# davawen/Simple-Raytracer

Measured on AMD Instinct MI355X. Metric: Mray/s at 1920x1080x1024spp, higher is better.
Workload: dtype f32; 1 GPU; BASELINE configs[1]: 7-shape sphere scene 1920x1080 1024spp; width=1920, height=1080, spp=1024, bounces=10, triangles=12, partition=single GPU, gather=none, mode=parity (fp-contract off, IEEE div/sqrt; canvas bit-identical to the CPU oracle)

## Files before the change

### include/srt_abi.h

```cpp
#ifndef SRT_ABI_H
#define SRT_ABI_H

#include "srt_types.h"

#ifdef __cplusplus
extern "C" {
#endif

typedef struct srt_tracer srt_tracer;

enum {
	SRT_OK = 0,
	SRT_ERR_INVALID = 1,
	SRT_ERR_HIP = 2,
	SRT_ERR_STATE = 3
};

typedef struct srt_counters {
	uint64_t paths;
	uint64_t rays;
	uint64_t sky;
	uint64_t tri_tests;
	uint64_t tri_pass_u;
	uint64_t nan_pixels;
// ... 254 lines not shown
int srt_group_read_bloom(srt_group *g, int level, float *rgba_out, size_t cap_pixels, int *w, int *h);
int srt_last_resolve_bloomed(const srt_tracer *t, int *bloomed);
int srt_group_last_resolve_bloomed(const srt_group *g, int *bloomed);

#define SRT_NOISE_EIGHTHS {0x1.000000p+0f, 0x1.172b84p+0f, 0x1.306fe0p+0f, 0x1.4bfdaep+0f, 0x1.6a09e6p+0f, 0x1.8ace54p+0f, 0x1.ae89fap+0f, 0x1.d5818ep+0f}
int srt_noise_defaults(srt_noise_params *out);
int srt_noise_check_host(const srt_noise_params *p);
int srt_noise_evaluate_host(const uint32_t hist[256], const uint32_t counts[3], uint32_t T, uint32_t P, const srt_noise_params *params, srt_noise_result *result);
int srt_set_noise_meter(srt_tracer *t, const srt_noise_params *p);
int srt_group_set_noise_meter(srt_group *g, const srt_noise_params *p);
int srt_meter_noise(srt_tracer *t);
int srt_group_meter_noise(srt_group *g);
int srt_poll_noise(srt_tracer *t, srt_noise_result *result, uint32_t hist[256], int *ready);
int srt_read_noise(srt_tracer *t, srt_noise_result *result, uint32_t hist[256]);
int srt_group_poll_noise(srt_group *g, srt_noise_result *result, uint32_t hist[256], int *ready);
int srt_group_read_noise(srt_group *g, srt_noise_result *result, uint32_t hist[256]);
int srt_resolve_noise_view(srt_tracer *t);
int srt_group_resolve_noise_view(srt_group *g);
int srt_group_read_noise_view(srt_group *g, uint8_t *argb_out);
int srt_render_until(srt_tracer *t, const srt_render_data *options, uint32_t time_stride, uint32_t max_dispatches, uint8_t *argb_out,
                     srt_noise_result *result, uint32_t *dispatches_done);
int srt_last_meter_ran(const srt_tracer *t, int *ran);
int srt_selftest_noise_meter(srt_tracer *t, const float *canvas_host, const float *moments_host, uint32_t num_pixels, uint32_t T, uint32_t P,
                             const srt_noise_params *params, uint32_t hist_out[256], uint32_t counts_out[3], uint8_t *view_out);


int srt_cast_rays(srt_tracer *t, const srt_ray *rays, size_t n, uint32_t flags, srt_ray_hit *hits);
int srt_cast_rays_device(srt_tracer *t, const void *rays_dev, size_t n, uint32_t flags, void *hits_dev);
int srt_pick(srt_tracer *t, const srt_render_data *options, const float *xy, size_t n, srt_ray_hit *hits);
int srt_group_cast_rays(srt_group *g, const srt_ray *rays, size_t n, uint32_t flags, srt_ray_hit *hits);
int srt_group_pick(srt_group *g, const srt_render_data *options, const float *xy, size_t n, srt_ray_hit *hits);
int srt_last_ray_query_ms(srt_tracer *t, float *ms);
int srt_ray_query_sizes(size_t out[2]);


int srt_occluded_rays(srt_tracer *t, const srt_ray *rays, size_t n, uint32_t flags, uint64_t *occluded, uint64_t *invalid );
int srt_occluded_rays_device(srt_tracer *t, const void *rays_dev, size_t n, uint32_t flags, void *occluded_dev, void *invalid_dev );
int srt_occluded_segments(srt_tracer *t, const srt_segment *segs, size_t n, uint64_t *occluded, uint64_t *invalid );
int srt_segment_rays(srt_tracer *t, const srt_segment *segs, size_t n, srt_ray *rays_out);
int srt_group_occluded_rays(srt_group *g, const srt_ray *rays, size_t n, uint32_t flags, uint64_t *occluded, uint64_t *invalid);
int srt_group_occluded_segments(srt_group *g, const srt_segment *segs, size_t n, uint64_t *occluded, uint64_t *invalid);
int srt_group_segment_rays(srt_group *g, const srt_segment *segs, size_t n, srt_ray *rays_out);
int srt_occlusion_sizes(size_t out[2]);

int srt_selftest_math(srt_tracer *t, uint32_t stride, uint64_t out[16]);

int srt_selftest_rare_lanes(srt_tracer *t, int what, const uint32_t *in, uint32_t waves, uint32_t *out_new, uint32_t *out_ref, uint64_t *mismatches);

int srt_selftest_plane_forms(srt_tracer *t, int what, const float planes[32], const float cam_org[3], const uint32_t *in, uint32_t waves,
                             uint32_t *out_new, uint32_t *out_ref, uint32_t *fast, uint64_t *mismatches);

int srt_selftest_diffuse_bounce(srt_tracer *t, const uint32_t *in, uint32_t waves, uint32_t *out_new, uint32_t *out_ref, uint32_t *fast, uint64_t *mismatches);

int srt_selection_defaults(srt_selection_params *out);
int srt_selection_check_host(const srt_selection_params *p);
int srt_selection_sizes(size_t out[1]);
int srt_selection_alpha_table_host(const srt_selection_params *p, uint8_t *table, size_t cap, int *radius);
int srt_set_selection(srt_tracer *t, const srt_selection_params *p, const uint32_t *shapes, size_t n);
int srt_group_set_selection(srt_group *g, const srt_selection_params *p, const uint32_t *shapes, size_t n);
int srt_render_ids(srt_tracer *t, const srt_render_data *options);
int srt_read_id_pass(srt_tracer *t, uint32_t *shape, uint32_t *triangle, int32_t *material, size_t cap_pixels, int *w, int *h);
int srt_group_read_id_pass(srt_group *g, uint32_t *shape, uint32_t *triangle, int32_t *material, size_t cap_pixels, int *w, int *h);
int srt_read_selection_alpha(srt_tracer *t, uint8_t *alpha, size_t cap_pixels);
int srt_last_resolve_selected(const srt_tracer *t, int *applied, int *id_pass_ran);
int srt_group_last_resolve_selected(const srt_group *g, int *applied, int *id_pass_ran);

const char *srt_version(void);

#ifdef __cplusplus
}
#endif

#endif
```

### simple-raytracer_amd/csrc/frame.hip

```cpp
#include <hip/hip_runtime.h>

#include "device_math.h"
#include "tonemap.h"

namespace {
__device__ __forceinline__ float add_lum2(float s2, float r, float g, float b) {
	const float l = lum(r, g, b);
	return s2 + l * l;
}
}
template <bool MOMENTS>
__global__ __launch_bounds__(256) void srt_reduce_kernel(const ReduceParams p) {
	const uint32_t q = blockIdx.x * blockDim.x + threadIdx.x;
	if (q == 0u && p.queue_reset) *p.queue_reset = 0ull;
	if (q >= p.num_pixels) return;
	f3 c = mk(0.f, 0.f, 0.f);
	float s2 = 0.f;
	float4 *run = reinterpret_cast<float4 *>(p.running) + q;
	if (!p.first_batch) {
		float4 v = *run;
		c = mk(v.x, v.y, v.z);
		if (MOMENTS) s2 = v.w;
	}
	const uint32_t n = p.batch_samples;
	const float *__restrict__ r = p.radiance + (size_t)q * n * 3u;
	uint32_t k = 0;
	if ((n & 3u) == 0u) {
		const float4 *__restrict__ r4 = reinterpret_cast<const float4 *>(r);
#ifndef SRT_REDUCE_DEPTH
#define SRT_REDUCE_DEPTH 4
#endif
		for (; k + 4 * SRT_REDUCE_DEPTH <= n; k += 4 * SRT_REDUCE_DEPTH) {
			float4 v[3 * SRT_REDUCE_DEPTH];
#pragma unroll
			for (int i = 0; i < 3 * SRT_REDUCE_DEPTH; i++) v[i] = r4[i];
			r4 += 3 * SRT_REDUCE_DEPTH;
#pragma unroll
			for (int i = 0; i < 3 * SRT_REDUCE_DEPTH; i += 3) {
				const float4 a = v[i], b = v[i + 1], d = v[i + 2];
				c = c + mk(a.x, a.y, a.z);
				if (MOMENTS) s2 = add_lum2(s2, a.x, a.y, a.z);
				c = c + mk(a.w, b.x, b.y);
				if (MOMENTS) s2 = add_lum2(s2, a.w, b.x, b.y);
				c = c + mk(b.z, b.w, d.x);
				if (MOMENTS) s2 = add_lum2(s2, b.z, b.w, d.x);
				c = c + mk(d.y, d.z, d.w);
				if (MOMENTS) s2 = add_lum2(s2, d.y, d.z, d.w);
			}
		}
		for (; k < n; k += 4) {
			const float4 a = r4[0], b = r4[1], d = r4[2];
			r4 += 3;
			c = c + mk(a.x, a.y, a.z);
			if (MOMENTS) s2 = add_lum2(s2, a.x, a.y, a.z);
			c = c + mk(a.w, b.x, b.y);
			if (MOMENTS) s2 = add_lum2(s2, a.w, b.x, b.y);
			c = c + mk(b.z, b.w, d.x);
			if (MOMENTS) s2 = add_lum2(s2, b.z, b.w, d.x);
			c = c + mk(d.y, d.z, d.w);
			if (MOMENTS) s2 = add_lum2(s2, d.y, d.z, d.w);
		}
	} else {
		for (; k < n; k++) {
			c = c + mk(r[3 * k], r[3 * k + 1], r[3 * k + 2]);
			if (MOMENTS) s2 = add_lum2(s2, r[3 * k], r[3 * k + 1], r[3 * k + 2]);
		}
	}
	if (p.last_batch) {
		c = c / (float)p.num_samples;
		float4 *out = reinterpret_cast<float4 *>(p.canvas) + q;
		float4 o = *out;
		o.x += c.x;
		o.y += c.y;
		o.z += c.z;
		*out = o;
		if (c.x != c.x || c.y != c.y || c.z != c.z) atomicAdd(&p.counters[SRT_CTR_NAN], 1ull);
		if (!MOMENTS && p.argb) {
			const float n = (float)p.num_steps;
			const float r = sqrt_ieee(aces1(o.x / n)), g = sqrt_ieee(aces1(o.y / n)), b = sqrt_ieee(aces1(o.z / n));
			reinterpret_cast<uint32_t *>(p.argb)[q] = 255u | (to_uchar(r * 255.0f) << 8) | (to_uchar(g * 255.0f) << 16) | (to_uchar(b * 255.0f) << 24);
		}
		if (MOMENTS) p.moments[q] += s2 / (float)p.num_samples;
	} else {
		*run = make_float4(c.x, c.y, c.z, MOMENTS ? s2 : 0.f);
	}
}

__global__ __launch_bounds__(256) void srt_prepass_kernel(const PrepassParams p) {
	const int si = blockIdx.y;
	if (si >= p.num_shapes) return;
	const srt_shape *sh = p.shapes + si;
	if (sh->type != SRT_SHAPE_MODEL) return;
	const srt_model *m = &sh->shape.model;
	const uint32_t n = m->num_triangles;
	const uint32_t base = p.wtri_offset[si];
	for (uint32_t s = blockIdx.x * blockDim.x + threadIdx.x; s < n; s += gridDim.x * blockDim.x) {
		const uint32_t j = p.order ? p.order[base + s] : s;
		const srt_triangle *t = p.triangles + (m->triangle_index + j);
		f3 p0 = mat_by_vec(m->transform, ld3(t->vertices[0].pos), 1.0f);
		f3 p1 = mat_by_vec(m->transform, ld3(t->vertices[1].pos), 1.0f);
		f3 p2 = mat_by_vec(m->transform, ld3(t->vertices[2].pos), 1.0f);
		f3 e1 = p1 - p0, e2 = p2 - p0;
		float *w = p.order ? p.wtris + (size_t)(p.dest[base + s] >> 2) * 32u + (p.dest[base + s] & 3u) * SRT_BVH_TRI_FLOATS
		                   : p.wtris + (size_t)(base + s) * SRT_WTRI_FLOATS;
		w[0] = p0.x, w[1] = p0.y, w[2] = p0.z;
		w[3] = e1.x, w[4] = e1.y, w[5] = e1.z;
		w[6] = e2.x, w[7] = e2.y, w[8] = e2.z;
		if (p.order) p.wtris[(size_t)(p.dest[base + s] >> 2) * 32u + SRT_BVH_LEAF_J + (p.dest[base + s] & 3u)] = dm_u2f(j);
	}
}


__global__ __launch_bounds__(256) void srt_resolve_kernel(const ResolveParams p) {
	const float4 *__restrict__ canvas = reinterpret_cast<const float4 *>(p.canvas);
	uint32_t *__restrict__ out = reinterpret_cast<uint32_t *>(p.argb);
	const float n = (float)p.num_steps;
	for (uint32_t i = blockIdx.x * blockDim.x + threadIdx.x; i < p.num_pixels; i += gridDim.x * blockDim.x) {
		float4 c = canvas[i];
		float r = sqrt_ieee(aces1(c.x / n));
		float g = sqrt_ieee(aces1(c.y / n));
		float b = sqrt_ieee(aces1(c.z / n));
		out[i] = 255u | (to_uchar(r * 255.0f) << 8) | (to_uchar(g * 255.0f) << 16) | (to_uchar(b * 255.0f) << 24);
	}
}

void srt_launch_reduce(const ReduceParams &p, void *stream) {
	if (p.num_pixels == 0) return;
	hipLaunchKernelGGL(srt_reduce_kernel<false>, dim3((p.num_pixels + 255) / 256), dim3(256), 0, (hipStream_t)stream, p);
}

void srt_launch_prepass(const PrepassParams &p, uint64_t max_tris_per_model, void *stream) {
	if (p.num_shapes <= 0 || max_tris_per_model == 0) return;
	unsigned gx = (unsigned)((max_tris_per_model + 255) / 256);
	if (gx > 4096) gx = 4096;
	dim3 grid(gx, (unsigned)p.num_shapes), block(256);
	hipLaunchKernelGGL(srt_prepass_kernel, grid, block, 0, (hipStream_t)stream, p);
}

void srt_launch_resolve(const ResolveParams &p, void *stream) {
	if (p.num_pixels == 0) return;
	unsigned gx = (p.num_pixels + 255) / 256;
	if (gx > 4096) gx = 4096;
	hipLaunchKernelGGL(srt_resolve_kernel, dim3(gx), dim3(256), 0, (hipStream_t)stream, p);
}

void srt_launch_reduce_moments(const ReduceParams &p, void *stream) {
	if (p.num_pixels == 0) return;
	hipLaunchKernelGGL(srt_reduce_kernel<true>, dim3((p.num_pixels + 255) / 256), dim3(256), 0, (hipStream_t)stream, p);
}
```

### simple-raytracer_amd/csrc/srt_abi.hip

```cpp
#include <hip/hip_runtime.h>

#include <cstdlib>
#include <cstring>
#include <new>
#include <string>
#include <vector>

#include "../../include/srt_abi.h"
#include "detmath.h"
#include "device_types.h"

#include "scene_prep.h"
#include "srt_internal.h"
#include "trace_plan.h"

namespace {

thread_local std::string g_create_error;

int num_blocks(int height, int rpb) { return (height + rpb - 1) / rpb; }

int clear_canvas_impl(srt_tracer *t) {
	const int rc = srt_temporal_commit(t);
	if (rc) return rc;
// ... 1004 lines not shown
	if (!planes || !cam_org || !in || !out_new || !out_ref || !fast || !mismatches || what < 0 || what > 1 || waves == 0 || waves > 65536u)
		return fail(t, SRT_ERR_INVALID, "srt_selftest_plane_forms: bad arguments");
	SRT_HIP(t, hipSetDevice(t->device));
	const size_t lanes = (size_t)waves * 64u, in_bytes = lanes * 8u * sizeof(uint32_t), out_bytes = lanes * 2u * sizeof(uint32_t), fast_bytes = (size_t)waves * sizeof(uint32_t);
	char *d = nullptr;
	SRT_HIP(t, hipMalloc(reinterpret_cast<void **>(&d), in_bytes + 2 * out_bytes + sizeof(unsigned long long) + fast_bytes));
	uint32_t *d_in = reinterpret_cast<uint32_t *>(d), *d_new = reinterpret_cast<uint32_t *>(d + in_bytes), *d_ref = reinterpret_cast<uint32_t *>(d + in_bytes + out_bytes);
	unsigned long long *d_bad = reinterpret_cast<unsigned long long *>(d + in_bytes + 2 * out_bytes), h_bad = 0;
	uint32_t *d_fast = reinterpret_cast<uint32_t *>(d + in_bytes + 2 * out_bytes + sizeof(unsigned long long));
	hipError_t e = hipMemcpyAsync(d_in, in, in_bytes, hipMemcpyHostToDevice, t->stream);
	if (e == hipSuccess) e = hipMemsetAsync(d_new, 0, 2 * out_bytes + sizeof(unsigned long long) + fast_bytes, t->stream);
	if (e == hipSuccess) {
		srt_launch_selftest_plane_forms(what, planes, cam_org, d_in, waves, d_new, d_ref, d_fast, d_bad, t->stream);
		e = hipGetLastError();
	}
	if (e == hipSuccess) e = hipMemcpyAsync(out_new, d_new, out_bytes, hipMemcpyDeviceToHost, t->stream);
	if (e == hipSuccess) e = hipMemcpyAsync(out_ref, d_ref, out_bytes, hipMemcpyDeviceToHost, t->stream);
	if (e == hipSuccess) e = hipMemcpyAsync(fast, d_fast, fast_bytes, hipMemcpyDeviceToHost, t->stream);
	if (e == hipSuccess) e = hipMemcpyAsync(&h_bad, d_bad, sizeof h_bad, hipMemcpyDeviceToHost, t->stream);
	if (e == hipSuccess) e = hipStreamSynchronize(t->stream);
	(void)hipFree(d);
	if (e != hipSuccess) return fail(t, SRT_ERR_HIP, std::string("srt_selftest_plane_forms: ") + hipGetErrorString(e));
	*mismatches = h_bad;
	return SRT_OK;
}

int srt_selftest_diffuse_bounce(srt_tracer *t, const uint32_t *in, uint32_t waves, uint32_t *out_new, uint32_t *out_ref, uint32_t *fast, uint64_t *mismatches) {
	if (!t) return SRT_ERR_INVALID;
	if (!in || !out_new || !out_ref || !fast || !mismatches || waves == 0 || waves > 65536u) return fail(t, SRT_ERR_INVALID, "srt_selftest_diffuse_bounce: bad arguments");
	SRT_HIP(t, hipSetDevice(t->device));
	const size_t lanes = (size_t)waves * 64u, in_bytes = lanes * 20u * sizeof(uint32_t), out_bytes = lanes * 8u * sizeof(uint32_t), fast_bytes = (size_t)waves * sizeof(uint32_t);
	char *d = nullptr;
	SRT_HIP(t, hipMalloc(reinterpret_cast<void **>(&d), in_bytes + 2 * out_bytes + sizeof(unsigned long long) + fast_bytes));
	uint32_t *d_in = reinterpret_cast<uint32_t *>(d), *d_new = reinterpret_cast<uint32_t *>(d + in_bytes), *d_ref = reinterpret_cast<uint32_t *>(d + in_bytes + out_bytes);
	unsigned long long *d_bad = reinterpret_cast<unsigned long long *>(d + in_bytes + 2 * out_bytes), h_bad = 0;
	uint32_t *d_fast = reinterpret_cast<uint32_t *>(d + in_bytes + 2 * out_bytes + sizeof(unsigned long long));
	hipError_t e = hipMemcpyAsync(d_in, in, in_bytes, hipMemcpyHostToDevice, t->stream);
	if (e == hipSuccess) e = hipMemsetAsync(d_new, 0, 2 * out_bytes + sizeof(unsigned long long) + fast_bytes, t->stream);
	if (e == hipSuccess) {
		srt_launch_selftest_diffuse_bounce(d_in, waves, d_new, d_ref, d_fast, d_bad, t->stream);
		e = hipGetLastError();
	}
	if (e == hipSuccess) e = hipMemcpyAsync(out_new, d_new, out_bytes, hipMemcpyDeviceToHost, t->stream);
	if (e == hipSuccess) e = hipMemcpyAsync(out_ref, d_ref, out_bytes, hipMemcpyDeviceToHost, t->stream);
	if (e == hipSuccess) e = hipMemcpyAsync(fast, d_fast, fast_bytes, hipMemcpyDeviceToHost, t->stream);
	if (e == hipSuccess) e = hipMemcpyAsync(&h_bad, d_bad, sizeof h_bad, hipMemcpyDeviceToHost, t->stream);
	if (e == hipSuccess) e = hipStreamSynchronize(t->stream);
	(void)hipFree(d);
	if (e != hipSuccess) return fail(t, SRT_ERR_HIP, std::string("srt_selftest_diffuse_bounce: ") + hipGetErrorString(e));
	*mismatches = h_bad;
	return SRT_OK;
}

int srt_debug_counters(srt_tracer *t, uint64_t out[18]) {
	if (!t || !out) return SRT_ERR_INVALID;
	SRT_HIP(t, hipSetDevice(t->device));
	std::vector<unsigned long long> w;
	if (const int rc = read_wave_counters(t, w, nullptr)) return rc;
	for (int k = 0; k < 18; k++) out[k] = 0;
	for (size_t i = 0; i < (size_t)2 * SRT_WAVE_CTR_SLOTS; i++) {
		for (int k = 0; k < 8; k++) out[k] += w[i * SRT_WAVE_CTR_STRIDE + k];
		for (int k = 8; k < 16; k++) out[k + 2] += w[i * SRT_WAVE_CTR_STRIDE + k];
	}
	out[8] = (uint64_t)t->last_waves_per_cu;
	out[9] = (uint64_t)t->last_grid;
	return SRT_OK;
}

int srt_debug_region_counters(srt_tracer *t, uint64_t *out, int capacity, int *written) {
	if (!t || !out || !written || capacity < 0) return SRT_ERR_INVALID;
	*written = 0;
#ifdef SRT_REGION_COUNT
	SRT_HIP(t, hipSetDevice(t->device));
	std::vector<unsigned long long> w;
	if (const int rc = read_wave_counters(t, w, nullptr)) return rc;
	const int n = capacity < 2 * SRT_REGION_MAX ? capacity : 2 * SRT_REGION_MAX;
	for (int k = 0; k < n; k++) out[k] = 0;
	for (size_t i = 0; i < (size_t)2 * SRT_WAVE_CTR_SLOTS; i++)
		for (int k = 0; k < n; k++) out[k] += w[i * SRT_WAVE_CTR_STRIDE + 16 + k];
	*written = n;
#endif
	return SRT_OK;
}

int srt_set_count_triangles(srt_tracer *t, int enable) {
	if (!t) return SRT_ERR_INVALID;
	t->count_tris = enable != 0;
	return SRT_OK;
}

}

TraceParams srt_trace_params_for_query(const srt_tracer *t, const srt_render_data *options) { return trace_params_of(t, options, false); }
```

### simple-raytracer_amd/tracer.py

```python
import ctypes as C
from pathlib import Path

import numpy as np

from . import build as B
from . import records as R

PKG = Path(__file__).resolve().parent
import os

LIB_PATH = Path(os.environ["SRT_LIB"]) if os.environ.get("SRT_LIB") else PKG / "lib" / "libsrt_hip.so"

ABI_SYMBOLS = [
    "srt_create", "srt_destroy", "srt_last_error", "srt_set_skybox", "srt_update_scene", "srt_clear_canvas",
    "srt_render", "srt_render_async", "srt_trace", "srt_set_radiance_budget", "srt_resolve", "srt_resolve_external", "srt_synchronize", "srt_read_canvas", "srt_read_argb",
    "srt_get_counters", "srt_set_count_triangles", "srt_reset_counters", "srt_last_kernel_ms", "srt_set_kernel_timers", "srt_last_trace_kernel_ms", "srt_last_trace_launches",
    "srt_device_buffers", "srt_bind_canvas", "srt_bind_stream", "srt_set_partition",
    "srt_partition_owned_rows", "srt_partition_padded_rows", "srt_partition_global_row",
    "srt_partition_unpermute", "srt_selftest_math", "srt_selftest_rare_lanes", "srt_version", "srt_set_acceleration", "srt_acceleration_info", "srt_bvh_build_host", "srt_bvh_wide_host", "srt_debug_counters", "srt_debug_region_counters",
    "srt_comm_unique_id", "srt_comm_init", "srt_gather", "srt_resolve_gathered", "srt_gathered_buffers", "srt_read_gathered",
    "srt_group_create", "srt_group_destroy", "srt_group_last_error", "srt_group_size", "srt_group_tracer", "srt_group_set_skybox",
    "srt_group_set_acceleration", "srt_group_update_scene", "srt_group_clear_canvas", "srt_group_trace_and_gather", "srt_group_render",
    "srt_group_read_canvas", "srt_group_get_counters", "srt_render_pipelined", "srt_pipeline_flush", "srt_unpermute_device",
    "srt_denoise_defaults", "srt_set_denoise", "srt_resolve_denoised", "srt_read_denoised", "srt_read_denoise_inputs",
    "srt_temporal_defaults", "srt_set_denoise_temporal", "srt_reset_denoise_history", "srt_read_denoise_history",
    "srt_set_denoise_object_motion", "srt_read_denoise_shape_ids", "srt_read_denoise_motion", "srt_motion_table_host",
    "srt_set_denoise_vertex_motion", "srt_read_denoise_triangle_ids", "srt_read_denoise_vertex_tables", "srt_motion_table_deform_host",
    "srt_set_textures", "srt_set_material_textures", "srt_set_triangle_uvs", "srt_last_trace_textured", "srt_plane_frame_host",
    "srt_texture_check_host", "srt_group_set_textures", "srt_group_set_material_textures", "srt_group_set_triangle_uvs",
    "srt_last_trace_class", "srt_bernoulli_threshold_host",
    "srt_last_trace_plane_form", "srt_plane_axis_code_host", "srt_selftest_plane_forms", "srt_selftest_diffuse_bounce",
    "srt_set_triangle_materials", "srt_group_set_triangle_materials", "srt_triangle_materials_check_host",
    "srt_group_set_denoise", "srt_group_set_denoise_temporal", "srt_group_reset_denoise_history", "srt_group_resolve_denoised",
    "srt_group_read_denoised", "srt_group_read_denoise_inputs", "srt_group_read_denoise_history", "srt_partition_planes_floats",
    "srt_unpermute_planes_device",
    "srt_set_denoise_demodulation", "srt_group_set_denoise_demodulation", "srt_last_filter_demodulated",
    "srt_group_last_filter_demodulated",
    "srt_set_denoise_spatial_variance", "srt_group_set_denoise_spatial_variance", "srt_last_filter_spatial_variance",
    "srt_group_last_filter_spatial_variance",
    "srt_set_denoise_history_illumination", "srt_group_set_denoise_history_illumination", "srt_last_setup_history_illumination",
    "srt_group_last_setup_history_illumination",
    "srt_set_denoise_history_clamp", "srt_group_set_denoise_history_clamp", "srt_last_setup_history_clamp",
    "srt_group_last_setup_history_clamp", "srt_read_denoise_history_bounds",
    "srt_set_denoise_history_feedback", "srt_group_set_denoise_history_feedback", "srt_last_filter_history_feedback",
    "srt_group_last_filter_history_feedback",
    "srt_bvh_refit_wide_host", "srt_set_acceleration_refit", "srt_group_set_acceleration_refit", "srt_acceleration_refit_info",
    "srt_last_refit_kernel_ms", "srt_read_bvh_blocks", "srt_bvh_wide_order_host",
    "srt_set_acceleration_deform", "srt_group_set_acceleration_deform", "srt_acceleration_deform_info",
    "srt_bvh_refit_deformed_wide_host", "srt_bvh_wide_cost_host",
    "srt_set_acceleration_build", "srt_group_set_acceleration_build", "srt_acceleration_build_info", "srt_last_build_kernel_ms",
    "srt_bvh_morton_order_host", "srt_bvh_morton_wide_host",
    "srt_set_acceleration_build_order", "srt_group_set_acceleration_build_order", "srt_bvh_median_order_host", "srt_bvh_median_wide_host",
    "srt_exposure_defaults", "srt_exposure_check_host", "srt_set_exposure", "srt_group_set_exposure", "srt_reset_exposure",
    "srt_group_reset_exposure", "srt_read_exposure", "srt_group_read_exposure", "srt_last_resolve_exposed",
    "srt_group_last_resolve_exposed",
    "srt_bloom_defaults", "srt_bloom_check_host", "srt_set_bloom", "srt_group_set_bloom", "srt_read_bloom", "srt_group_read_bloom",
    "srt_last_resolve_bloomed", "srt_group_last_resolve_bloomed",
    "srt_noise_defaults", "srt_noise_check_host", "srt_noise_evaluate_host", "srt_set_noise_meter", "srt_group_set_noise_meter",
    "srt_meter_noise", "srt_group_meter_noise", "srt_poll_noise", "srt_group_poll_noise", "srt_read_noise", "srt_group_read_noise",
    "srt_resolve_noise_view", "srt_group_resolve_noise_view", "srt_group_read_noise_view", "srt_render_until", "srt_last_meter_ran",
    "srt_selftest_noise_meter",
    "srt_cast_rays", "srt_cast_rays_device", "srt_pick", "srt_group_cast_rays", "srt_group_pick", "srt_last_ray_query_ms",
    "srt_ray_query_sizes",
    "srt_occluded_rays", "srt_occluded_rays_device", "srt_occluded_segments", "srt_segment_rays", "srt_group_occluded_rays",
    "srt_group_occluded_segments", "srt_group_segment_rays", "srt_occlusion_sizes",
    "srt_selection_defaults", "srt_selection_check_host", "srt_selection_sizes", "srt_selection_alpha_table_host", "srt_set_selection",
    "srt_group_set_selection", "srt_render_ids", "srt_read_id_pass", "srt_group_read_id_pass", "srt_read_selection_alpha",
    "srt_last_resolve_selected", "srt_group_last_resolve_selected",
]

ACCEL_NONE, ACCEL_BVH = 0, 1
REFIT_HOST, REFIT_DEVICE = 0, 1
DEFORM_REBUILD, DEFORM_REFIT = 0, 1
BUILD_HOST, BUILD_DEVICE = 0, 1
BUILD_ORDER_MORTON, BUILD_ORDER_MEDIAN = 0, 1
BUILD_LOCAL = 1024
MOTION_STATIC, MOTION_MOVED, MOTION_NO_HISTORY, MOTION_DEFORMED = 0, 1, 2, 3
MOTION_WORDS = 22
NO_SHAPE = 0xFFFFFFFF
FILTER_LINEAR, FILTER_NEAREST = 0, 1
MAX_TEXTURES = 64


class TextureDesc(C.Structure):
# ... 598 lines not shown
        lib.srt_read_denoise_triangle_ids.argtypes = [vp, vp, vp]
        lib.srt_read_denoise_vertex_tables.argtypes = [vp, vp, vp, sz, C.POINTER(sz)]
        lib.srt_motion_table_deform_host.argtypes = [vp, sz, vp, sz, vp, sz, vp] * 2 + [vp, C.POINTER(C.c_int)]
    if hasattr(lib, "srt_set_denoise_demodulation"):
        lib.srt_set_denoise_demodulation.argtypes = [vp, C.c_int]
        lib.srt_group_set_denoise_demodulation.argtypes = [vp, C.c_int]
        lib.srt_last_filter_demodulated.argtypes = [vp, C.POINTER(C.c_int)]
        lib.srt_group_last_filter_demodulated.argtypes = [vp, C.POINTER(C.c_int)]
    if hasattr(lib, "srt_set_denoise_spatial_variance"):
        lib.srt_set_denoise_spatial_variance.argtypes = [vp, C.c_uint32]
        lib.srt_group_set_denoise_spatial_variance.argtypes = [vp, C.c_uint32]
        lib.srt_last_filter_spatial_variance.argtypes = [vp, C.POINTER(C.c_int)]
        lib.srt_group_last_filter_spatial_variance.argtypes = [vp, C.POINTER(C.c_int)]
    if hasattr(lib, "srt_set_denoise_history_illumination"):
        lib.srt_set_denoise_history_illumination.argtypes = [vp, C.c_int]
        lib.srt_group_set_denoise_history_illumination.argtypes = [vp, C.c_int]
        lib.srt_last_setup_history_illumination.argtypes = [vp]
        lib.srt_group_last_setup_history_illumination.argtypes = [vp]
    if hasattr(lib, "srt_set_denoise_history_clamp"):
        lib.srt_set_denoise_history_clamp.argtypes = [vp, C.c_float]
        lib.srt_group_set_denoise_history_clamp.argtypes = [vp, C.c_float]
        lib.srt_last_setup_history_clamp.argtypes = [vp]
        lib.srt_group_last_setup_history_clamp.argtypes = [vp]
        lib.srt_read_denoise_history_bounds.argtypes = [vp, vp, vp]
    if hasattr(lib, "srt_set_denoise_history_feedback"):
        lib.srt_set_denoise_history_feedback.argtypes = [vp, C.c_int]
        lib.srt_group_set_denoise_history_feedback.argtypes = [vp, C.c_int]
        lib.srt_last_filter_history_feedback.argtypes = [vp]
        lib.srt_group_last_filter_history_feedback.argtypes = [vp]
    if hasattr(lib, "srt_set_textures"):
        lib.srt_set_textures.argtypes = [vp, vp, sz]
        lib.srt_set_material_textures.argtypes = [vp, vp, sz]
        lib.srt_set_triangle_uvs.argtypes = [vp, vp, sz]
        lib.srt_last_trace_textured.argtypes = [vp, C.POINTER(C.c_int)]
        lib.srt_plane_frame_host.argtypes = [vp, vp, vp]
        lib.srt_texture_check_host.argtypes = [vp, sz, vp, sz, C.c_longlong, sz]
        lib.srt_group_set_textures.argtypes = [vp, vp, sz]
        lib.srt_group_set_material_textures.argtypes = [vp, vp, sz]
        lib.srt_group_set_triangle_uvs.argtypes = [vp, vp, sz]
    if hasattr(lib, "srt_set_triangle_materials"):
        lib.srt_set_triangle_materials.argtypes = [vp, vp, sz]
        lib.srt_group_set_triangle_materials.argtypes = [vp, vp, sz]
        lib.srt_triangle_materials_check_host.argtypes = [vp, sz, sz, sz]
    if hasattr(lib, "srt_last_trace_class"):
        lib.srt_last_trace_class.argtypes = [vp, C.POINTER(C.c_int)]
    if hasattr(lib, "srt_last_trace_plane_form"):
        lib.srt_last_trace_plane_form.argtypes = [vp, C.POINTER(C.c_int)]
        lib.srt_plane_axis_code_host.argtypes = [vp, vp, C.POINTER(C.c_int)]
        u32p = C.POINTER(C.c_uint32)
        lib.srt_selftest_plane_forms.argtypes = [vp, i, vp, vp, u32p, C.c_uint32, u32p, u32p, u32p, C.POINTER(C.c_uint64)]
    if hasattr(lib, "srt_selftest_diffuse_bounce"):
        u32p = C.POINTER(C.c_uint32)
        lib.srt_selftest_diffuse_bounce.argtypes = [vp, u32p, C.c_uint32, u32p, u32p, u32p, C.POINTER(C.c_uint64)]
    if hasattr(lib, "srt_bernoulli_threshold_host"):
        lib.srt_bernoulli_threshold_host.argtypes = [C.c_float, C.POINTER(C.c_uint64)]
    if hasattr(lib, "srt_set_exposure"):
        fp, u32p = C.POINTER(C.c_float), C.POINTER(C.c_uint32)
        lib.srt_exposure_defaults.argtypes = [C.POINTER(ExposureParams)]
        lib.srt_exposure_check_host.argtypes = [C.POINTER(ExposureParams)]
        for pre in ("srt_", "srt_group_"):
            getattr(lib, pre + "set_exposure").argtypes = [vp, C.POINTER(ExposureParams)]
            getattr(lib, pre + "reset_exposure").argtypes = [vp]
            getattr(lib, pre + "read_exposure").argtypes = [vp, fp, fp, u32p, u32p]
            getattr(lib, pre + "last_resolve_exposed").argtypes = [vp, C.POINTER(C.c_int)]
    if hasattr(lib, "srt_set_bloom"):
        ip = C.POINTER(C.c_int)
        lib.srt_bloom_defaults.argtypes = [C.POINTER(BloomParams)]
        lib.srt_bloom_check_host.argtypes = [C.POINTER(BloomParams)]
        for pre in ("srt_", "srt_group_"):
            getattr(lib, pre + "set_bloom").argtypes = [vp, C.POINTER(BloomParams)]
            getattr(lib, pre + "read_bloom").argtypes = [vp, C.c_int, C.POINTER(C.c_float), C.c_size_t, ip, ip]
            getattr(lib, pre + "last_resolve_bloomed").argtypes = [vp, ip]
    if hasattr(lib, "srt_set_noise_meter"):
        ip, u32p, fp = C.POINTER(C.c_int), C.POINTER(C.c_uint32), C.POINTER(C.c_float)
        npp, nrp = C.POINTER(NoiseParams), C.POINTER(NoiseResult)
        lib.srt_noise_defaults.argtypes = [npp]
        lib.srt_noise_check_host.argtypes = [npp]
        lib.srt_noise_evaluate_host.argtypes = [u32p, u32p, C.c_uint32, C.c_uint32, npp, nrp]
        for pre in ("srt_", "srt_group_"):
            getattr(lib, pre + "set_noise_meter").argtypes = [vp, npp]
            getattr(lib, pre + "meter_noise").argtypes = [vp]
            getattr(lib, pre + "poll_noise").argtypes = [vp, nrp, u32p, ip]
            getattr(lib, pre + "read_noise").argtypes = [vp, nrp, u32p]
            getattr(lib, pre + "resolve_noise_view").argtypes = [vp]
        lib.srt_group_read_noise_view.argtypes = [vp, vp]
        lib.srt_render_until.argtypes = [vp, vp, C.c_uint32, C.c_uint32, vp, nrp, u32p]
        lib.srt_last_meter_ran.argtypes = [vp, ip]
        lib.srt_selftest_noise_meter.argtypes = [vp, fp, fp, C.c_uint32, C.c_uint32, C.c_uint32, npp, u32p, u32p, vp]
    if hasattr(lib, "srt_cast_rays"):
        for pre in ("srt_", "srt_group_"):
            getattr(lib, pre + "cast_rays").argtypes = [vp, vp, sz, C.c_uint32, vp]
            getattr(lib, pre + "pick").argtypes = [vp, vp, vp, sz, vp]
        lib.srt_cast_rays_device.argtypes = [vp, vp, sz, C.c_uint32, vp]
        lib.srt_last_ray_query_ms.argtypes = [vp, C.POINTER(C.c_float)]
        lib.srt_ray_query_sizes.argtypes = [C.POINTER(sz)]
        sizes = (sz * 2)()
        assert lib.srt_ray_query_sizes(sizes) == 0 and (sizes[0], sizes[1]) == (R.RAY.itemsize, R.RAY_HIT.itemsize), tuple(sizes)
    if hasattr(lib, "srt_occluded_rays"):
        for pre in ("srt_", "srt_group_"):
            getattr(lib, pre + "occluded_rays").argtypes = [vp, vp, sz, C.c_uint32, vp, vp]
            getattr(lib, pre + "occluded_segments").argtypes = [vp, vp, sz, vp, vp]
            getattr(lib, pre + "segment_rays").argtypes = [vp, vp, sz, vp]
        lib.srt_occluded_rays_device.argtypes = [vp, vp, sz, C.c_uint32, vp, vp]
        lib.srt_occlusion_sizes.argtypes = [C.POINTER(sz)]
        sizes = (sz * 2)()
        assert lib.srt_occlusion_sizes(sizes) == 0 and (sizes[0], sizes[1]) == (R.SEGMENT.itemsize, 8), tuple(sizes)
# ... 431 lines not shown
        self._check(self.lib.srt_acceleration_refit_info(self._h, out))
        return dict(zip(("models", "inner_blocks", "launches"), (int(v) for v in out)))

    def last_refit_kernel_ms(self):
        a = C.c_float()
        self._check(self.lib.srt_last_refit_kernel_ms(self._h, C.byref(a)))
        return a.value

    def read_bvh_blocks(self):
        n = C.c_size_t(0)
        self._check(self.lib.srt_read_bvh_blocks(self._h, None, 0, C.byref(n)))
        blocks = np.zeros((n.value, 32), np.uint32)
        self._check(self.lib.srt_read_bvh_blocks(self._h, _ptr(blocks), len(blocks), C.byref(n)))
        return blocks

    def selftest_math(self, stride=1):
        out = (C.c_uint64 * 16)()
        self._check(self.lib.srt_selftest_math(self._h, stride, out))
        return [int(v) for v in out]

    def selftest_rare_lanes(self, what, words):
        words = np.ascontiguousarray(words, np.uint32)
        assert words.ndim == 2 and words.shape[1] == 8 and words.shape[0] % 64 == 0
        new, ref, bad = np.zeros((words.shape[0], 4), np.uint32), np.zeros((words.shape[0], 4), np.uint32), C.c_uint64()
        u32p = C.POINTER(C.c_uint32)
        self._check(self.lib.srt_selftest_rare_lanes(self._h, int(what), words.ctypes.data_as(u32p), words.shape[0] // 64,
                                                     new.ctypes.data_as(u32p), ref.ctypes.data_as(u32p), C.byref(bad)))
        return new, ref, int(bad.value)

    def selftest_plane_forms(self, what, planes, cam_org, words):
        words = np.ascontiguousarray(words, np.uint32)
        planes = np.ascontiguousarray(planes, np.float32).reshape(32)
        cam_org = np.ascontiguousarray(cam_org, np.float32).reshape(3)
        assert words.ndim == 2 and words.shape[1] == 8 and words.shape[0] % 64 == 0
        waves = words.shape[0] // 64
        new, ref = np.zeros((words.shape[0], 2), np.uint32), np.zeros((words.shape[0], 2), np.uint32)
        fast, bad = np.zeros(waves, np.uint32), C.c_uint64()
        u32p = C.POINTER(C.c_uint32)
        self._check(self.lib.srt_selftest_plane_forms(self._h, int(what), _ptr(planes), _ptr(cam_org), words.ctypes.data_as(u32p), waves,
                                                      new.ctypes.data_as(u32p), ref.ctypes.data_as(u32p), fast.ctypes.data_as(u32p), C.byref(bad)))
        return new, ref, fast, int(bad.value)

    def selftest_diffuse_bounce(self, words):
        words = np.ascontiguousarray(words, np.uint32)
        assert words.ndim == 2 and words.shape[1] == 20 and words.shape[0] % 64 == 0
        waves = words.shape[0] // 64
        new, ref = np.zeros((words.shape[0], 8), np.uint32), np.zeros((words.shape[0], 8), np.uint32)
        fast, bad = np.zeros(waves, np.uint32), C.c_uint64()
        u32p = C.POINTER(C.c_uint32)
        self._check(self.lib.srt_selftest_diffuse_bounce(self._h, words.ctypes.data_as(u32p), waves, new.ctypes.data_as(u32p),
                                                         ref.ctypes.data_as(u32p), fast.ctypes.data_as(u32p), C.byref(bad)))
        return new, ref, fast, int(bad.value)

    def set_kernel_timers(self, enable=True):
        self._check(self.lib.srt_set_kernel_timers(self._h, int(bool(enable))))

    def last_kernel_ms(self):
        a, b = C.c_float(), C.c_float()
        self._check(self.lib.srt_last_kernel_ms(self._h, C.byref(a), C.byref(b)))
        return a.value, b.value

    def last_trace_launches(self):
        n, o = C.c_int(0), C.c_int(0)
        self.lib.srt_last_trace_launches.argtypes = [C.c_void_p, C.POINTER(C.c_int), C.POINTER(C.c_int)]
        self._check(self.lib.srt_last_trace_launches(self._h, C.byref(n), C.byref(o)))
        return n.value, bool(o.value)

    def last_trace_kernel_ms(self):
        a = C.c_float()
        self._check(self.lib.srt_last_trace_kernel_ms(self._h, C.byref(a)))
        return a.value

    def device_buffers(self):
        cp, cb, ap, ab = C.c_void_p(), C.c_size_t(), C.c_void_p(), C.c_size_t()
        self._check(self.lib.srt_device_buffers(self._h, C.byref(cp), C.byref(cb), C.byref(ap), C.byref(ab)))
        return cp.value, cb.value, ap.value, ab.value

    def bind_canvas(self, device_ptr, nbytes):
        self._check(self.lib.srt_bind_canvas(self._h, C.c_void_p(device_ptr), nbytes))

    def bind_stream(self, hip_stream):
        self._check(self.lib.srt_bind_stream(self._h, C.c_void_p(hip_stream)))

    @staticmethod
    def comm_unique_id():
        buf = C.create_string_buffer(128)
        if load_library().srt_comm_unique_id(buf):
            raise SrtError(load_library().srt_last_error(None).decode())
        return buf.raw

    def comm_init(self, unique_id, rank, world):
        self._check(self.lib.srt_comm_init(self._h, C.c_char_p(unique_id), rank, world))

    def gather(self, root=0):
        self._check(self.lib.srt_gather(self._h, root))

    def resolve_gathered(self, ticks_stopped):
        self._check(self.lib.srt_resolve_gathered(self._h, ticks_stopped))

    def gathered_buffers(self):
        cp, ap = C.c_void_p(), C.c_void_p()
        self._check(self.lib.srt_gathered_buffers(self._h, C.byref(cp), C.byref(ap)))
        return cp.value, ap.value

    def read_gathered(self, canvas=True, argb=False):
        c = np.zeros((self.height, self.width, 4), np.float32) if canvas else None
# ... 253 lines not shown
```

Measured before the change: 101,700 Mray/s.

## Add LDS-tiled coalesced radiance reduce kernel with per-wave transpose

Adds a tiled reduce kernel. Each wavefront loads chunks of 16 samples for its 64 pixels with coalesced 16-byte loads, transposes them through padded LDS, and then sums per pixel. The existing kernel has each thread read its own contiguous sample stream, which gives strided, uncoalesced global access. The new path costs extra LDS traffic, wave barriers and register pressure, and it runs only when the batch sample count is a multiple of 4 and at least 16. A selftest entry point is also added to check the new path against expected results.

```diff
diff --git a/include/srt_abi.h b/include/srt_abi.h
--- a/include/srt_abi.h
+++ b/include/srt_abi.h
@@ -330,6 +330,9 @@
 
 int srt_selftest_diffuse_bounce(srt_tracer *t, const uint32_t *in, uint32_t waves, uint32_t *out_new, uint32_t *out_ref, uint32_t *fast, uint64_t *mismatches);
 
+int srt_selftest_reduce(srt_tracer *t, const float *radiance, uint32_t num_pixels, const uint32_t *batch_samples, uint32_t num_batches, int32_t num_samples,
+                        int moments, float *canvas, uint32_t canvas_pixels, float *moments_io, uint64_t *nan_pixels);
+
 int srt_selection_defaults(srt_selection_params *out);
 int srt_selection_check_host(const srt_selection_params *p);
 int srt_selection_sizes(size_t out[1]);
diff --git a/simple-raytracer_amd/csrc/frame.hip b/simple-raytracer_amd/csrc/frame.hip
--- a/simple-raytracer_amd/csrc/frame.hip
+++ b/simple-raytracer_amd/csrc/frame.hip
@@ -8,64 +8,19 @@
 	const float l = lum(r, g, b);
 	return s2 + l * l;
 }
-}
-template <bool MOMENTS>
-__global__ __launch_bounds__(256) void srt_reduce_kernel(const ReduceParams p) {
-	const uint32_t q = blockIdx.x * blockDim.x + threadIdx.x;
-	if (q == 0u && p.queue_reset) *p.queue_reset = 0ull;
-	if (q >= p.num_pixels) return;
-	f3 c = mk(0.f, 0.f, 0.f);
-	float s2 = 0.f;
-	float4 *run = reinterpret_cast<float4 *>(p.running) + q;
-	if (!p.first_batch) {
-		float4 v = *run;
-		c = mk(v.x, v.y, v.z);
-		if (MOMENTS) s2 = v.w;
-	}
-	const uint32_t n = p.batch_samples;
-	const float *__restrict__ r = p.radiance + (size_t)q * n * 3u;
-	uint32_t k = 0;
-	if ((n & 3u) == 0u) {
-		const float4 *__restrict__ r4 = reinterpret_cast<const float4 *>(r);
-#ifndef SRT_REDUCE_DEPTH
-#define SRT_REDUCE_DEPTH 4
-#endif
-		for (; k + 4 * SRT_REDUCE_DEPTH <= n; k += 4 * SRT_REDUCE_DEPTH) {
-			float4 v[3 * SRT_REDUCE_DEPTH];
-#pragma unroll
-			for (int i = 0; i < 3 * SRT_REDUCE_DEPTH; i++) v[i] = r4[i];
-			r4 += 3 * SRT_REDUCE_DEPTH;
-#pragma unroll
-			for (int i = 0; i < 3 * SRT_REDUCE_DEPTH; i += 3) {
-				const float4 a = v[i], b = v[i + 1], d = v[i + 2];
-				c = c + mk(a.x, a.y, a.z);
-				if (MOMENTS) s2 = add_lum2(s2, a.x, a.y, a.z);
-				c = c + mk(a.w, b.x, b.y);
-				if (MOMENTS) s2 = add_lum2(s2, a.w, b.x, b.y);
-				c = c + mk(b.z, b.w, d.x);
-				if (MOMENTS) s2 = add_lum2(s2, b.z, b.w, d.x);
-				c = c + mk(d.y, d.z, d.w);
-				if (MOMENTS) s2 = add_lum2(s2, d.y, d.z, d.w);
-			}
-		}
-		for (; k < n; k += 4) {
-			const float4 a = r4[0], b = r4[1], d = r4[2];
-			r4 += 3;
-			c = c + mk(a.x, a.y, a.z);
-			if (MOMENTS) s2 = add_lum2(s2, a.x, a.y, a.z);
-			c = c + mk(a.w, b.x, b.y);
-			if (MOMENTS) s2 = add_lum2(s2, a.w, b.x, b.y);
-			c = c + mk(b.z, b.w, d.x);
-			if (MOMENTS) s2 = add_lum2(s2, b.z, b.w, d.x);
-			c = c + mk(d.y, d.z, d.w);
-			if (MOMENTS) s2 = add_lum2(s2, d.y, d.z, d.w);
-		}
-	} else {
-		for (; k < n; k++) {
-			c = c + mk(r[3 * k], r[3 * k + 1], r[3 * k + 2]);
-			if (MOMENTS) s2 = add_lum2(s2, r[3 * k], r[3 * k + 1], r[3 * k + 2]);
-		}
-	}
+template <bool MOMENTS>
+__device__ __forceinline__ void add_samples4(f3 &c, float &s2, const float4 a, const float4 b, const float4 d) {
+	c = c + mk(a.x, a.y, a.z);
+	if (MOMENTS) s2 = add_lum2(s2, a.x, a.y, a.z);
+	c = c + mk(a.w, b.x, b.y);
+	if (MOMENTS) s2 = add_lum2(s2, a.w, b.x, b.y);
+	c = c + mk(b.z, b.w, d.x);
+	if (MOMENTS) s2 = add_lum2(s2, b.z, b.w, d.x);
+	c = c + mk(d.y, d.z, d.w);
+	if (MOMENTS) s2 = add_lum2(s2, d.y, d.z, d.w);
+}
+template <bool MOMENTS>
+__device__ __forceinline__ void reduce_finish(const ReduceParams &p, uint32_t q, f3 c, float s2) {
 	if (p.last_batch) {
 		c = c / (float)p.num_samples;
 		float4 *out = reinterpret_cast<float4 *>(p.canvas) + q;
@@ -82,9 +37,135 @@
 		}
 		if (MOMENTS) p.moments[q] += s2 / (float)p.num_samples;
 	} else {
-		*run = make_float4(c.x, c.y, c.z, MOMENTS ? s2 : 0.f);
-	}
-}
+		reinterpret_cast<float4 *>(p.running)[q] = make_float4(c.x, c.y, c.z, MOMENTS ? s2 : 0.f);
+	}
+}
+}
+template <bool MOMENTS>
+__global__ __launch_bounds__(256) void srt_reduce_kernel(const ReduceParams p) {
+	const uint32_t q = blockIdx.x * blockDim.x + threadIdx.x;
+	if (q == 0u && p.queue_reset) *p.queue_reset = 0ull;
+	if (q >= p.num_pixels) return;
+	f3 c = mk(0.f, 0.f, 0.f);
+	float s2 = 0.f;
+	float4 *run = reinterpret_cast<float4 *>(p.running) + q;
+	if (!p.first_batch) {
+		float4 v = *run;
+		c = mk(v.x, v.y, v.z);
+		if (MOMENTS) s2 = v.w;
+	}
+	const uint32_t n = p.batch_samples;
+	const float *__restrict__ r = p.radiance + (size_t)q * n * 3u;
+	uint32_t k = 0;
+	if ((n & 3u) == 0u) {
+		const float4 *__restrict__ r4 = reinterpret_cast<const float4 *>(r);
+#ifndef SRT_REDUCE_DEPTH
+#define SRT_REDUCE_DEPTH 4
+#endif
+		for (; k + 4 * SRT_REDUCE_DEPTH <= n; k += 4 * SRT_REDUCE_DEPTH) {
+			float4 v[3 * SRT_REDUCE_DEPTH];
+#pragma unroll
+			for (int i = 0; i < 3 * SRT_REDUCE_DEPTH; i++) v[i] = r4[i];
+			r4 += 3 * SRT_REDUCE_DEPTH;
+#pragma unroll
+			for (int i = 0; i < 3 * SRT_REDUCE_DEPTH; i += 3) {
+				const float4 a = v[i], b = v[i + 1], d = v[i + 2];
+				add_samples4<MOMENTS>(c, s2, a, b, d);
+			}
+		}
+		for (; k < n; k += 4) {
+			const float4 a = r4[0], b = r4[1], d = r4[2];
+			r4 += 3;
+			add_samples4<MOMENTS>(c, s2, a, b, d);
+		}
+	} else {
+		for (; k < n; k++) {
+			c = c + mk(r[3 * k], r[3 * k + 1], r[3 * k + 2]);
+			if (MOMENTS) s2 = add_lum2(s2, r[3 * k], r[3 * k + 1], r[3 * k + 2]);
+		}
+	}
+	reduce_finish<MOMENTS>(p, q, c, s2);
+}
+
+namespace {
+constexpr uint32_t RT_SAMPLES = 16u;
+constexpr uint32_t RT_VEC = RT_SAMPLES * 3u / 4u;
+constexpr uint32_t RT_STRIDE = RT_VEC + 1u;
+constexpr uint32_t RT_WAVE_WORDS = 64u * RT_STRIDE;
+typedef float reduce_vf4 __attribute__((ext_vector_type(4)));
+__device__ __forceinline__ float4 ld16(const float4 *p) {
+	const reduce_vf4 t = *reinterpret_cast<const reduce_vf4 *>(p);
+	return make_float4(t.x, t.y, t.z, t.w);
+}
+__device__ __forceinline__ void wave_lds_sync() {
+	__builtin_amdgcn_fence(__ATOMIC_RELEASE, "wavefront");
+	__builtin_amdgcn_wave_barrier();
+	__builtin_amdgcn_fence(__ATOMIC_ACQUIRE, "wavefront");
+}
+}
+template <bool MOMENTS>
+__global__ __launch_bounds__(256) void srt_reduce_tiled_kernel(const ReduceParams p) {
+	__shared__ float4 tiles[4u * RT_WAVE_WORDS];
+	const uint32_t lane = threadIdx.x & 63u;
+	const uint32_t q0 = blockIdx.x * 256u + (threadIdx.x & ~63u);
+	const uint32_t q = q0 + lane;
+	if (q == 0u && p.queue_reset) *p.queue_reset = 0ull;
+	if (q0 >= p.num_pixels) return;
+	const uint32_t live = p.num_pixels - q0;
+	const bool own = lane < live;
+	float4 *__restrict__ tile = tiles + (threadIdx.x >> 6) * RT_WAVE_WORDS;
+	f3 c = mk(0.f, 0.f, 0.f);
+	float s2 = 0.f;
+	if (!p.first_batch && own) {
+		const float4 v = reinterpret_cast<const float4 *>(p.running)[q];
+		c = mk(v.x, v.y, v.z);
+		if (MOMENTS) s2 = v.w;
+	}
+	const uint32_t n = p.batch_samples;
+	const uint32_t pv = n / 4u * 3u;
+	const float4 *__restrict__ base = reinterpret_cast<const float4 *>(p.radiance + (size_t)q0 * n * 3u);
+	uint32_t src[RT_VEC], dst[RT_VEC];
+#pragma unroll
+	for (uint32_t i = 0; i < RT_VEC; i++) {
+		const uint32_t e = 64u * i + lane, j = e / RT_VEC, m = e - j * RT_VEC;
+		src[i] = (j < live ? j : live - 1u) * pv + m, dst[i] = j * RT_STRIDE + m;
+	}
+	const uint32_t trips = n / RT_SAMPLES;
+	float4 v[RT_VEC];
+#pragma unroll
+	for (uint32_t i = 0; i < RT_VEC; i++) v[i] = ld16(base + src[i]);
+	const auto stage = [&]() {
+#pragma unroll
+		for (uint32_t i = 0; i < RT_VEC; i++) tile[dst[i]] = v[i];
+		wave_lds_sync();
+	};
+	const auto add_up = [&]() {
+		float4 w[RT_VEC];
+#pragma unroll
+		for (uint32_t i = 0; i < RT_VEC; i++) w[i] = tile[lane * RT_STRIDE + i];
+		wave_lds_sync();
+#pragma unroll
+		for (uint32_t i = 0; i < RT_VEC; i += 3) add_samples4<MOMENTS>(c, s2, w[i], w[i + 1], w[i + 2]);
+	};
+	for (uint32_t t = 1; t < trips; t++) {
+		stage();
+		base += RT_VEC;
+#pragma unroll
+		for (uint32_t i = 0; i < RT_VEC; i++) v[i] = ld16(base + src[i]);
+		add_up();
+	}
+	stage();
+	add_up();
+	if (!own) return;
+	const float4 *__restrict__ r4 = reinterpret_cast<const float4 *>(p.radiance + (size_t)q * n * 3u) + trips * RT_VEC;
+	for (uint32_t k = trips * RT_SAMPLES; k < n; k += 4) {
+		const float4 a = r4[0], b = r4[1], d = r4[2];
+		r4 += 3;
+		add_samples4<MOMENTS>(c, s2, a, b, d);
+	}
+	reduce_finish<MOMENTS>(p, q, c, s2);
+}
+static bool reduce_tiled_ok(const ReduceParams &p) { return (p.batch_samples & 3u) == 0u && p.batch_samples >= RT_SAMPLES; }
 
 __global__ __launch_bounds__(256) void srt_prepass_kernel(const PrepassParams p) {
 	const int si = blockIdx.y;
@@ -126,7 +207,8 @@
 
 void srt_launch_reduce(const ReduceParams &p, void *stream) {
 	if (p.num_pixels == 0) return;
-	hipLaunchKernelGGL(srt_reduce_kernel<false>, dim3((p.num_pixels + 255) / 256), dim3(256), 0, (hipStream_t)stream, p);
+	if (reduce_tiled_ok(p)) hipLaunchKernelGGL(srt_reduce_tiled_kernel<false>, dim3((p.num_pixels + 255) / 256), dim3(256), 0, (hipStream_t)stream, p);
+	else hipLaunchKernelGGL(srt_reduce_kernel<false>, dim3((p.num_pixels + 255) / 256), dim3(256), 0, (hipStream_t)stream, p);
 }
 
 void srt_launch_prepass(const PrepassParams &p, uint64_t max_tris_per_model, void *stream) {
@@ -146,5 +228,6 @@
 
 void srt_launch_reduce_moments(const ReduceParams &p, void *stream) {
 	if (p.num_pixels == 0) return;
-	hipLaunchKernelGGL(srt_reduce_kernel<true>, dim3((p.num_pixels + 255) / 256), dim3(256), 0, (hipStream_t)stream, p);
-}
+	if (reduce_tiled_ok(p)) hipLaunchKernelGGL(srt_reduce_tiled_kernel<true>, dim3((p.num_pixels + 255) / 256), dim3(256), 0, (hipStream_t)stream, p);
+	else hipLaunchKernelGGL(srt_reduce_kernel<true>, dim3((p.num_pixels + 255) / 256), dim3(256), 0, (hipStream_t)stream, p);
+}
diff --git a/simple-raytracer_amd/csrc/srt_abi.hip b/simple-raytracer_amd/csrc/srt_abi.hip
--- a/simple-raytracer_amd/csrc/srt_abi.hip
+++ b/simple-raytracer_amd/csrc/srt_abi.hip
@@ -1080,6 +1080,61 @@
 	return SRT_OK;
 }
 
+int srt_selftest_reduce(srt_tracer *t, const float *radiance, uint32_t num_pixels, const uint32_t *batch_samples, uint32_t num_batches, int32_t num_samples,
+                        int moments, float *canvas, uint32_t canvas_pixels, float *moments_io, uint64_t *nan_pixels) {
+	if (!t) return SRT_ERR_INVALID;
+	if (!radiance || !batch_samples || !canvas || !nan_pixels || (moments && !moments_io) || num_pixels == 0 || canvas_pixels < num_pixels || num_batches == 0 ||
+	    num_batches > 64u)
+		return fail(t, SRT_ERR_INVALID, "srt_selftest_reduce: bad arguments");
+	size_t floats = 0, largest = 0;
+	for (uint32_t b = 0; b < num_batches; b++) {
+		if (batch_samples[b] == 0 || batch_samples[b] > (1u << 20)) return fail(t, SRT_ERR_INVALID, "srt_selftest_reduce: bad batch");
+		const size_t f = (size_t)num_pixels * batch_samples[b] * 3u;
+		floats += f, largest = f > largest ? f : largest;
+	}
+	if (floats > ((size_t)1 << 28)) return fail(t, SRT_ERR_INVALID, "srt_selftest_reduce: too large");
+	SRT_HIP(t, hipSetDevice(t->device));
+	const size_t rad_bytes = (largest * sizeof(float) + 255u) & ~(size_t)255u, px_bytes = (((size_t)canvas_pixels * 16u) + 255u) & ~(size_t)255u;
+	char *d = nullptr;
+	SRT_HIP(t, hipMalloc(reinterpret_cast<void **>(&d), rad_bytes + 3 * px_bytes + SRT_CTR_COUNT * sizeof(unsigned long long)));
+	ReduceParams rp;
+	rp.radiance = reinterpret_cast<const float *>(d);
+	rp.running = reinterpret_cast<float *>(d + rad_bytes);
+	rp.canvas = reinterpret_cast<float *>(d + rad_bytes + px_bytes);
+	float *d_mom = reinterpret_cast<float *>(d + rad_bytes + 2 * px_bytes);
+	rp.counters = reinterpret_cast<unsigned long long *>(d + rad_bytes + 3 * px_bytes);
+	rp.num_pixels = num_pixels;
+	rp.num_samples = num_samples;
+	rp.queue_reset = nullptr;
+	rp.argb = nullptr;
+	if (moments) rp.moments = d_mom;
+	rp.num_steps = 1;
+	unsigned long long h_ctr[SRT_CTR_COUNT] = {};
+	hipError_t e = hipMemsetAsync(d + rad_bytes, 0, 3 * px_bytes + sizeof h_ctr, t->stream);
+	if (e == hipSuccess) e = hipMemcpyAsync(rp.canvas, canvas, (size_t)canvas_pixels * 16u, hipMemcpyHostToDevice, t->stream);
+	if (e == hipSuccess && moments) e = hipMemcpyAsync(d_mom, moments_io, (size_t)num_pixels * sizeof(float), hipMemcpyHostToDevice, t->stream);
+	const float *src = radiance;
+	for (uint32_t b = 0; b < num_batches && e == hipSuccess; b++) {
+		const size_t f = (size_t)num_pixels * batch_samples[b] * 3u;
+		e = hipMemcpyAsync(d, src, f * sizeof(float), hipMemcpyHostToDevice, t->stream);
+		src += f;
+		if (e != hipSuccess) break;
+		rp.batch_samples = batch_samples[b];
+		rp.first_batch = b == 0, rp.last_batch = b + 1 == num_batches;
+		if (moments) srt_launch_reduce_moments(rp, t->stream);
+		else srt_launch_reduce(rp, t->stream);
+		e = hipGetLastError();
+	}
+	if (e == hipSuccess) e = hipMemcpyAsync(canvas, rp.canvas, (size_t)canvas_pixels * 16u, hipMemcpyDeviceToHost, t->stream);
+	if (e == hipSuccess && moments) e = hipMemcpyAsync(moments_io, d_mom, (size_t)num_pixels * sizeof(float), hipMemcpyDeviceToHost, t->stream);
+	if (e == hipSuccess) e = hipMemcpyAsync(h_ctr, rp.counters, sizeof h_ctr, hipMemcpyDeviceToHost, t->stream);
+	if (e == hipSuccess) e = hipStreamSynchronize(t->stream);
+	(void)hipFree(d);
+	if (e != hipSuccess) return fail(t, SRT_ERR_HIP, std::string("srt_selftest_reduce: ") + hipGetErrorString(e));
+	*nan_pixels = h_ctr[SRT_CTR_NAN];
+	return SRT_OK;
+}
+
 int srt_debug_counters(srt_tracer *t, uint64_t out[18]) {
 	if (!t || !out) return SRT_ERR_INVALID;
 	SRT_HIP(t, hipSetDevice(t->device));
diff --git a/simple-raytracer_amd/tracer.py b/simple-raytracer_amd/tracer.py
--- a/simple-raytracer_amd/tracer.py
+++ b/simple-raytracer_amd/tracer.py
@@ -29,7 +29,7 @@
     "srt_set_textures", "srt_set_material_textures", "srt_set_triangle_uvs", "srt_last_trace_textured", "srt_plane_frame_host",
     "srt_texture_check_host", "srt_group_set_textures", "srt_group_set_material_textures", "srt_group_set_triangle_uvs",
     "srt_last_trace_class", "srt_bernoulli_threshold_host",
-    "srt_last_trace_plane_form", "srt_plane_axis_code_host", "srt_selftest_plane_forms", "srt_selftest_diffuse_bounce",
+    "srt_last_trace_plane_form", "srt_plane_axis_code_host", "srt_selftest_plane_forms", "srt_selftest_diffuse_bounce", "srt_selftest_reduce",
     "srt_set_triangle_materials", "srt_group_set_triangle_materials", "srt_triangle_materials_check_host",
     "srt_group_set_denoise", "srt_group_set_denoise_temporal", "srt_group_reset_denoise_history", "srt_group_resolve_denoised",
     "srt_group_read_denoised", "srt_group_read_denoise_inputs", "srt_group_read_denoise_history", "srt_partition_planes_floats",
@@ -734,6 +734,9 @@
     if hasattr(lib, "srt_selftest_diffuse_bounce"):
         u32p = C.POINTER(C.c_uint32)
         lib.srt_selftest_diffuse_bounce.argtypes = [vp, u32p, C.c_uint32, u32p, u32p, u32p, C.POINTER(C.c_uint64)]
+    if hasattr(lib, "srt_selftest_reduce"):
+        fp, u32p = C.POINTER(C.c_float), C.POINTER(C.c_uint32)
+        lib.srt_selftest_reduce.argtypes = [vp, fp, C.c_uint32, u32p, C.c_uint32, C.c_int32, i, fp, C.c_uint32, fp, C.POINTER(C.c_uint64)]
     if hasattr(lib, "srt_bernoulli_threshold_host"):
         lib.srt_bernoulli_threshold_host.argtypes = [C.c_float, C.POINTER(C.c_uint64)]
     if hasattr(lib, "srt_set_exposure"):
@@ -1271,6 +1274,22 @@
                                                          ref.ctypes.data_as(u32p), fast.ctypes.data_as(u32p), C.byref(bad)))
         return new, ref, fast, int(bad.value)
 
+    def selftest_reduce(self, batches, num_samples, canvas, moments=None):
+        batches = [np.ascontiguousarray(b, np.float32) for b in batches]
+        pixels = batches[0].shape[0]
+        assert all(b.ndim == 3 and b.shape[0] == pixels and b.shape[2] == 3 for b in batches)
+        counts = np.array([b.shape[1] for b in batches], np.uint32)
+        radiance = np.concatenate([b.reshape(-1) for b in batches])
+        canvas = np.array(canvas, np.float32, order="C")
+        assert canvas.ndim == 2 and canvas.shape[1] == 4 and canvas.shape[0] >= pixels
+        mom = None if moments is None else np.array(moments, np.float32, order="C").reshape(pixels)
+        nan = C.c_uint64()
+        fp = C.POINTER(C.c_float)
+        self._check(self.lib.srt_selftest_reduce(self._h, radiance.ctypes.data_as(fp), pixels, counts.ctypes.data_as(C.POINTER(C.c_uint32)), len(batches),
+                                                 int(num_samples), int(mom is not None), canvas.ctypes.data_as(fp), canvas.shape[0],
+                                                 None if mom is None else mom.ctypes.data_as(fp), C.byref(nan)))
+        return canvas, mom, int(nan.value)
+
     def set_kernel_timers(self, enable=True):
         self._check(self.lib.srt_set_kernel_timers(self._h, int(bool(enable))))
 
```

Measured after the change: 102,200 Mray/s, median of 6. Within noise of the previous version (+0.5%).
